# jantonguirao/nvImageCodec

Hardware: AMD Instinct MI355X
Metric: images/sec, batched 1920x1080 4:2:0 baseline JPEG decode to interleaved RGB u8 (higher is better)
Workload: dtype int32

## Files before the change

nvimagecodec_amd/csrc/gpu_huffman.hip:

```cpp
#include <hip/hip_runtime.h>

#include "gpu_huffman.h"
#include "huffman_gpu_core.h"

namespace hipjpeg {

namespace {

constexpr int kThreads = 256;

constexpr int kRowShift = kSubseqWords == 32 ? 5 : kSubseqWords == 16 ? 4 : kSubseqWords == 64 ? 6 : -1;
static_assert(kRowShift > 0, "subsequences of 512, 1024 or 2048 bits");

#define HJ_LDS __attribute__((address_space(3)))
#define HJ_GLOBAL __attribute__((address_space(1)))
typedef unsigned int u32x4 __attribute__((ext_vector_type(4)));

struct KSlot {
    int16_t* base;
    uint32_t stride_y, stride_x;
};

constexpr int kStagedExtra = 2;
constexpr int kRowWords = kSubseqWords + kStagedExtra;
// ... 58 lines not shown
        *(HJ_GLOBAL uint16_t*)(records + (off + 2 * min(i, (uint32_t)kRecSlots))) = (uint16_t)(pos - bit0);
    }
};
__device__ __forceinline__ SlotRecorder slot_recorder(uint16_t* records, const HuffImage& im, uint32_t j)
{
    SlotRecorder r;
    r.records = (HJ_GLOBAL char*)records;
    r.off = (im.first_subseq + j) * (uint32_t)(2 * kRecShorts);
    r.bit0 = j * kSubseqBits;
    return r;
}
__device__ __forceinline__ void put_mark(const SlotRecorder& r, uint32_t begin, uint32_t limit, uint32_t total_bits, uint32_t z0, const SubseqState& st)
{
    *(HJ_GLOBAL uint16_t*)(r.records + (r.off + 2 * kRecMark)) = (uint16_t)record_mark(begin, min(limit, total_bits), z0, st);
}

template <class Env>
__device__ __forceinline__ SubseqState walk_subsequence(bool rst, bool record, const HuffGeom& geom, const Env& env, uint32_t begin, uint32_t limit, int z,
                                                        int k, uint32_t boundary0, const SlotRecorder& rec)
{
    if (rst) return decode_subsequence<true>(geom, env, begin, limit, z, k, boundary0);
    return record ? decode_subsequence<false>(geom, env, begin, limit, z, k, 0, rec) : decode_subsequence<false>(geom, env, begin, limit, z, k);
}

template <int ROWS>
__device__ __forceinline__ void stage_rows(uint32_t* lds_stream, const HuffImage& im, int first_row)
{
    const int t = threadIdx.x;
    const HJ_GLOBAL uint32_t* g = (const HJ_GLOBAL uint32_t*)im.stream;
    const int nwords = (int)im.stream_words;
    const int w0 = (first_row + t) * kSubseqWords;
    constexpr int kGroups = kSubseqWords / 4;
    u32x4 v[kGroups];
    typedef unsigned int u32x2 __attribute__((ext_vector_type(2)));
    u32x2 tail;
    {
        const int gd = w0 + kSubseqWords;
        const int gc = min(max(gd, 0), (nwords - 1) & ~1);
        const u32x2 x = *(const HJ_GLOBAL u32x2*)(g + gc);
        tail = (gd >= 0 && gd < nwords) ? x : u32x2{~0u, ~0u};
    }
#pragma unroll
    for (int i = 0; i < kGroups; i++) {
        const int gd = w0 + i * 4;
        const int gc = min(max(gd, 0), (nwords - 1) & ~3);
        const u32x4 x = *(const HJ_GLOBAL u32x4*)(g + gc);
        v[i] = (gd >= 0 && gd < nwords) ? x : u32x4{~0u, ~0u, ~0u, ~0u};
    }
    HJ_LDS uint32_t* dst = (HJ_LDS uint32_t*)lds_stream + t;
#pragma unroll
    for (int i = 0; i < kGroups; i++) {
        dst[(4 * i + 0) * ROWS] = __builtin_bswap32(v[i].x);
        dst[(4 * i + 1) * ROWS] = __builtin_bswap32(v[i].y);
        dst[(4 * i + 2) * ROWS] = __builtin_bswap32(v[i].z);
        dst[(4 * i + 3) * ROWS] = __builtin_bswap32(v[i].w);
    }
    dst[(kSubseqWords + 0) * ROWS] = __builtin_bswap32(tail.x);
    dst[(kSubseqWords + 1) * ROWS] = __builtin_bswap32(tail.y);
}

template <int THREADS>
__device__ __forceinline__ void stage_pool(HJ_LDS uint16_t* pool, const HuffImage& im)
{
    const HJ_GLOBAL u32x4* gp = (const HJ_GLOBAL u32x4*)im.pool;
    const uint32_t npool = im.pool_words >> 3;
    for (uint32_t i = threadIdx.x; i < npool; i += THREADS) {
        const u32x4 x = gp[i];
        HJ_LDS uint32_t* lp = reinterpret_cast<HJ_LDS uint32_t*>(pool) + i * 4;
        lp[0] = x.x;
        lp[1] = x.y;
        lp[2] = x.z;
        lp[3] = x.w;
    }
}

__device__ __forceinline__ void stage_constants(uint32_t* tsel, KSlot* kslot, uint32_t* zzw, const HuffImage& im, bool with_addresses)
{
    const int t = threadIdx.x;
    if (t < 10) {
        const HuffK hk = im.k[t];
        tsel[t] = ((uint32_t)hk.tdc * 2) | ((uint32_t)hk.tac * 2 << 16);
        if (with_addresses) {
            KSlot s;
            s.base = im.coef[hk.comp & 3] + (size_t)hk.blk0 * 64;
            s.stride_y = hk.stride_y;
            s.stride_x = hk.stride_x;
            kslot[t] = s;
        }
    }
    if (zzw && t >= 64 && t < 80) {
        constexpr uint8_t zz[64] = HJ_ZIGZAG_DEVICE_TABLE;
        const int i = (t - 64) * 4;
        zzw[t - 64] = ((uint32_t)zz[i] | ((uint32_t)zz[i + 1] << 8) | ((uint32_t)zz[i + 2] << 16) | ((uint32_t)zz[i + 3] << 24)) << 1;
    }
}

__device__ __forceinline__ DevEnv make_env(WgShared& sh, HJ_LDS uint16_t* pool, uint32_t first, const HuffGeom& geom)
{
    DevEnv env;
    env.stream_base = (uint32_t)(uintptr_t)(HJ_LDS uint32_t*)sh.stream;
    env.word0 = (first - 1) * kSubseqWords;
    env.row_addr = env.stream_base;
    env.row_word0 = env.word0;
    env.pool = (uint32_t)(uintptr_t)pool;
    env.tsel = (const HJ_LDS uint32_t*)sh.tsel;
    env.boundaries = geom.boundaries;
    env.num_boundaries = geom.num_boundaries;
    return env;
}

__device__ __forceinline__ int compact_tasks(WgShared& sh, bool has, int value, int* task)
{
    const int t = threadIdx.x;
    const unsigned long long mask = __ballot(has);
    const int below = __popcll(mask & ((1ull << (t & 63)) - 1));
    if ((t & 63) == 0) sh.wave_count[t >> 6] = (uint32_t)__popcll(mask);
    __syncthreads();
    int base = 0, n = 0;
#pragma unroll
    for (int w = 0; w < kSyncThreads / 64; w++) {
        const int c = (int)sh.wave_count[w];
        if (w < (t >> 6)) base += c;
        n += c;
    }
    if (has) sh.queue[base + below] = (uint32_t)value;
    __syncthreads();
    *task = t < n ? (int)sh.queue[t] : -1;
    return n;
}

constexpr int kGatherGroups = 64;
__global__ __launch_bounds__(kThreads) void gather_raw_kernel(const HuffImage* __restrict__ images, const HuffUnit* __restrict__ units, int nunits)
{
    for (int ui = blockIdx.x; ui < nunits; ui += gridDim.x) {
        const HuffUnit u = units[ui];
        const HuffImage& im = images[u.image];
        const uint8_t* src = im.raw_src;
        if (!src) continue;
        const uint32_t begin = u.first * (uint32_t)kDestuffChunk;
        if (begin >= im.raw_bytes) continue;
        const uint32_t n = min((uint32_t)kDestuffChunk, im.raw_bytes - begin);
        const uint8_t* s = src + begin;
        uint8_t* d = const_cast<uint8_t*>(im.raw) + begin;
        typedef u32x4 __attribute__((aligned(1))) u32x4_unaligned;
        for (uint32_t i = threadIdx.x * 16u; i + 16u <= n; i += kThreads * 16u) *(HJ_GLOBAL u32x4*)(d + i) = *(const HJ_GLOBAL u32x4_unaligned*)(s + i);
        const uint32_t tail = n & ~15u;
        if (threadIdx.x < (n & 15u)) d[tail + threadIdx.x] = s[tail + threadIdx.x];
    }
}


__device__ __forceinline__ uint32_t zero_bytes(uint32_t v) { return ~(((v & 0x7F7F7F7Fu) + 0x7F7F7F7Fu) | v | 0x7F7F7F7Fu); }

__device__ __forceinline__ uint32_t stuffed_mask(uint32_t x, uint32_t prev, uint32_t next)
{
    const uint32_t ff_before = zero_bytes(~((x << 8) | prev));
    const uint32_t rst_x = zero_bytes((x & 0xF8F8F8F8u) ^ 0xD0D0D0D0u);
    const uint32_t second = (zero_bytes(x) | rst_x) & ff_before;
    const uint32_t after = (x >> 8) | (next << 24);
    const uint32_t first = zero_bytes(~x) & zero_bytes((after & 0xF8F8F8F8u) ^ 0xD0D0D0D0u);
    return second | first;
}

__device__ __forceinline__ uint32_t lane_masks(const uint8_t* p, bool has_prev, uint32_t m[16], uint32_t x[16])
{
    const uint4* q = reinterpret_cast<const uint4*>(p);
    uint32_t prev = has_prev ? p[-1] : 0u;
    uint32_t n = 0;
#pragma unroll
    for (int i = 0; i < 4; i++) {
        const uint4 v = q[i];
        x[4 * i + 0] = v.x;
        x[4 * i + 1] = v.y;
        x[4 * i + 2] = v.z;
        x[4 * i + 3] = v.w;
    }
    const uint32_t behind = p[64];
#pragma unroll
    for (int i = 0; i < 16; i++) {
        m[i] = stuffed_mask(x[i], prev, i < 15 ? (x[i < 15 ? i + 1 : 15] & 0xFFu) : behind);
        prev = x[i] >> 24;
        n += __popc(m[i]);
    }
    return n;
}

__device__ __forceinline__ uint32_t wg_sum(uint32_t v, uint32_t* scratch )
{
    for (int off = 32; off > 0; off >>= 1) v += __shfl_xor(v, off);
    if ((threadIdx.x & 63) == 0) scratch[threadIdx.x >> 6] = v;
    __syncthreads();
    const uint32_t total = scratch[0] + scratch[1] + scratch[2] + scratch[3];
    __syncthreads();
    return total;
}

__global__ __launch_bounds__(kThreads) void destuff_count_kernel(const HuffImage* __restrict__ images, const HuffUnit* __restrict__ units,
                                                                 uint32_t* __restrict__ drops)
{
    __shared__ uint32_t scratch[4];
    const HuffUnit u = units[blockIdx.x];
    const HuffImage& im = images[u.image];
    const uint32_t off = u.first * kDestuffChunk + threadIdx.x * 64;
    uint32_t n = 0;
    if (off < im.raw_bytes) {
        uint32_t m[16], x[16];
        const uint32_t pieces = min(4u, (im.raw_bytes - off + 15) / 16);
        if (pieces == 4) {
            n = lane_masks(im.raw + off, off > 0, m, x);
        } else {
            uint32_t prev = off > 0 ? im.raw[off - 1] : 0u;
            const uint32_t* words = reinterpret_cast<const uint32_t*>(im.raw + off);
            for (uint32_t i = 0; i < pieces * 4; i++) {
                const uint32_t w = words[i];
                n += __popc(stuffed_mask(w, prev, words[i + 1] & 0xFFu));
                prev = w >> 24;
            }
        }
    }
    const uint32_t total = wg_sum(n, scratch);
    if (threadIdx.x == 0) drops[im.first_chunk + u.first] = total;
}

__global__ __launch_bounds__(kThreads) void destuff_compact_kernel(HuffImage* __restrict__ images, const HuffUnit* __restrict__ units,
                                                                   const uint32_t* __restrict__ drops, unsigned int* __restrict__ counters)
{
    if (blockIdx.x == 0 && threadIdx.x < 64 && counters) counters[threadIdx.x] = 0u;
    __shared__ uint32_t scratch[4];
    __shared__ uint32_t wave_base[4];
    __shared__ uint32_t buf[kDestuffChunk / 4 + kDestuffChunk / 64 + 8];
    HJ_LDS uint8_t* bytes = (HJ_LDS uint8_t*)buf;
    const HuffUnit u = units[blockIdx.x];
    HuffImage& im = images[u.image];
    const int t = threadIdx.x;
    const uint32_t raw_bytes = im.raw_bytes;
    uint32_t before = 0;
    for (uint32_t c = t; c < u.first; c += kThreads) before += drops[im.first_chunk + c];
    before = wg_sum(before, scratch);
    const uint32_t chunk_begin = u.first * kDestuffChunk;
    const uint32_t chunk_len = min((uint32_t)kDestuffChunk, raw_bytes - chunk_begin);
    const uint32_t gout = chunk_begin - before;
    const uint32_t a = gout & 3;

    {
        const uint32_t pieces = (chunk_len + 15) / 16;
        const HJ_GLOBAL u32x4* src = (const HJ_GLOBAL u32x4*)(im.raw + chunk_begin);
        constexpr uint32_t kPiecesPerLane = kDestuffChunk / 16 / kThreads;
        u32x4 v[kPiecesPerLane];
#pragma unroll
        for (uint32_t i = 0; i < kPiecesPerLane; i++) v[i] = src[min(i * kThreads + t, pieces - 1)];
#pragma unroll
        for (uint32_t i = 0; i < kPiecesPerLane; i++) {
            const uint32_t q = i * kThreads + t, g = q * 4 + (q >> 2);
            const u32x4 x = q < pieces ? v[i] : u32x4{0x01010101u, 0x01010101u, 0x01010101u, 0x01010101u};
            buf[g] = x.x;
            buf[g + 1] = x.y;
            buf[g + 2] = x.z;
            buf[g + 3] = x.w;
        }
    }
    const uint32_t before_chunk = chunk_begin > 0 ? im.raw[chunk_begin - 1] : 0u;
    const uint32_t behind_chunk = chunk_len == (uint32_t)kDestuffChunk ? im.raw[chunk_begin + kDestuffChunk] : 0x01u;
    __syncthreads();

    const uint32_t off = chunk_begin + t * 64;
    uint32_t x[16];
    unsigned long long kept = 0;
    uint32_t n = 0, len = 0;
    if (off < raw_bytes) {
        len = min(64u, raw_bytes - off);
        const uint32_t pieces = (len + 15) / 16;
        uint32_t prev = t > 0 ? buf[(t - 1) * 17 + 15] >> 24 : before_chunk;
#pragma unroll
        for (uint32_t i = 0; i < 16; i++) x[i] = i < pieces * 4 ? buf[t * 17 + i] : 0x01010101u;
        const uint32_t behind = pieces == 4 ? (t < kThreads - 1 ? buf[(t + 1) * 17] & 0xFFu : behind_chunk) : 0x01u;
#pragma unroll
        for (uint32_t i = 0; i < 16; i++) {
            uint32_t w = x[i];
            uint32_t d = stuffed_mask(w, prev, i < 15 ? (x[i < 15 ? i + 1 : 15] & 0xFFu) : behind);
            prev = w >> 24;
            n += __popc(d);
            if (len < 64) {
                const uint32_t in = len > i * 4 ? min(len - i * 4, 4u) : 0u;
                if (in < 4) d |= 0x80808080u << (8 * in);
            }
            w = (d & 0x80000000u) ? (w & 0x00FFFFFFu) : w;
            w = (d & 0x00800000u) ? ((w & 0xFFFFu) | ((w >> 8) & 0xFF0000u)) : w;
            w = (d & 0x00008000u) ? ((w & 0xFFu) | ((w >> 8) & 0xFFFF00u)) : w;
            w = (d & 0x00000080u) ? (w >> 8) : w;
            x[i] = w;
            kept |= (unsigned long long)(4 - __popc(d)) << (3 * i);
        }
    }
    uint32_t incl = n;
    for (int d = 1; d < 64; d <<= 1) {
        const uint32_t v = __shfl_up(incl, d);
        if ((t & 63) >= d) incl += v;
    }
    if ((t & 63) == 63) wave_base[t >> 6] = incl;
    __syncthreads();
    uint32_t excl = incl - n;
    for (int w = 0; w < (t >> 6); w++) excl += wave_base[w];
    const uint32_t chunk_drops = wave_base[0] + wave_base[1] + wave_base[2] + wave_base[3];
    auto padded = [](uint32_t k) { return k + ((k >> 6) << 2); };
    const uint32_t o0 = a + t * 64 - excl, cnt0 = o0 & 3;
    uint32_t o = o0 & ~3u, cnt = cnt0;
    unsigned long long acc = 0;
    if (len) {
#pragma unroll
        for (uint32_t i = 0; i < 16; i++) {
            acc |= (unsigned long long)x[i] << (8 * cnt);
            cnt += (uint32_t)(kept >> (3 * i)) & 7u;
            if (cnt >= 4) {
                buf[(o >> 2) + (o >> 6)] = (uint32_t)acc;
                acc >>= 32;
                cnt -= 4;
                o += 4;
            }
        }
    }
    __syncthreads();
    {
        const uint32_t from = o == (o0 & ~3u) ? cnt0 : 0u;
#pragma unroll
        for (uint32_t b = 0; b < 3; b++)
            if (b >= from && b < cnt) bytes[padded(o + b)] = (uint8_t)((uint32_t)acc >> (8 * b));
    }
    __syncthreads();
    const uint32_t n_out = chunk_len - chunk_drops;
    uint8_t* dst = const_cast<uint8_t*>(im.stream) + (gout - a);
    const uint32_t first_full = a ? 1 : 0, end_full = (a + n_out) / 4;
    for (uint32_t d = first_full + t; d < end_full; d += kThreads) reinterpret_cast<uint32_t*>(dst)[d] = buf[d + (d >> 4)];
    if (t < 4) {
        if (a && (uint32_t)t >= a && (uint32_t)t < a + n_out) dst[t] = bytes[padded((uint32_t)t)];
        const uint32_t tail = max(end_full, first_full) * 4 + t;
        if (tail >= a && tail < a + n_out && tail >= 4 * first_full) dst[tail] = bytes[padded(tail)];
    }
    if (chunk_begin + chunk_len == raw_bytes) {
        const uint32_t total = raw_bytes - before - chunk_drops;
        const uint32_t padded = ((total + 3) & ~3u) + kStreamSlackBytes;
        uint8_t* s = const_cast<uint8_t*>(im.stream);
        if (total + t < padded) s[total + t] = 0xFF;
        if (t == 0) {
            im.total_bits = total * 8;
            im.num_subseq = (total * 8 + kSubseqBits - 1) / kSubseqBits;
            im.stream_words = padded / 4;
        }
    }
}

__global__ __launch_bounds__(kSyncThreads) void huff_sync_kernel(const HuffImage* __restrict__ images, const HuffUnit* __restrict__ units,
                                                             unsigned long long* __restrict__ states, unsigned long long* __restrict__ incoming,
                                                             unsigned int* __restrict__ counters, int first_pass, int max_rounds,
                                                             uint16_t* __restrict__ tail_tasks, uint32_t* __restrict__ tail_count, uint16_t* records)
{
    __shared__ WgShared sh;
    extern __shared__ uint16_t dyn_pool[];
    HJ_LDS uint16_t* pool = (HJ_LDS uint16_t*)dyn_pool;
    const HuffUnit u = units[blockIdx.x];
    const HuffImage& im = images[u.image];
    const HuffGeom geom = make_geom(im);
    const uint32_t nsub = (geom.total_bits + kSubseqBits - 1) / kSubseqBits;
    if (u.first >= nsub) return;
    unsigned long long* gstate = states + im.first_subseq;
    const int t = threadIdx.x;
    const uint32_t j = u.first - 1 + t;
    const bool owner = t >= 1 && j < nsub;
    const int n_rows = (int)min((uint32_t)kSyncThreads, nsub - u.first + 1);
    unsigned long long in_state = 0;
    if (!first_pass) {
        in_state = u.first ? __hip_atomic_load(&gstate[u.first - 1], __ATOMIC_RELAXED, __HIP_MEMORY_SCOPE_AGENT) & kSyncMask : 0ull;
        if (in_state == incoming[blockIdx.x]) return;
    }
    stage_rows<kSyncThreads>(sh.stream, im, (int)u.first - 1);
    stage_pool<kSyncThreads>(pool, im);
    stage_constants(sh.tsel, nullptr, nullptr, im, false);
    __syncthreads();

    DevEnv env = make_env(sh, pool, u.first, geom);
    const bool rst = im.restart_interval != 0;
    unsigned long long old_global = ~0ull;
    int task = -1;
    const bool recording = !rst;
    if (first_pass) {
        const unsigned long long assumed = (unsigned long long)j * kSubseqBits;
        unsigned long long mine = 0;
        if (owner || (t == 0 && u.first > 0)) {
            const uint32_t bidx0 = boundary0_of(im, j);
            env.set_row(t);
            mine = pack_state(walk_subsequence(rst, false, geom, env, j * kSubseqBits, (j + 1) * kSubseqBits, 0, 0, bidx0, SlotRecorder()));
        }
        sh.end[t] = mine;
        __syncthreads();
        if (owner && ((sh.end[t - 1] & kSyncMask) != assumed || recording)) task = t;
    } else {
        if (owner) old_global = gstate[j];
        sh.end[t] = t == 0 ? in_state : old_global;
        if (t == 1) task = 1;
    }
    int rounds = 0;
    for (int round = 0; round < kSyncThreads + 2; round++) {
        __syncthreads();
        rounds++;
        unsigned long long now = 0;
        bool moved = false;
        if (task >= 0) {
            const SubseqState p = unpack_state(sh.end[task - 1]);
            env.set_row(task);
            const uint32_t jt = u.first - 1 + task;
            const SlotRecorder rec = slot_recorder(records, im, jt);
            const SubseqState st = walk_subsequence(rst, recording, geom, env, p.end_bit, (jt + 1) * kSubseqBits, p.zk & 255, p.zk >> 8, boundary0_of(im, jt), rec);
            if (recording) put_mark(rec, p.end_bit, (jt + 1) * kSubseqBits, geom.total_bits, p.zk & 255, st);
            now = pack_state(st);
            moved = ((now ^ sh.end[task]) & kSyncMask) != 0;
        }
        __syncthreads();
        if (task >= 0) sh.end[task] = now;
        const int pending = compact_tasks(sh, moved && task + 1 < n_rows, task + 1, &task);
        if (pending == 0 || rounds >= max_rounds) {
            if (tail_count) {
                if (t < pending) tail_tasks[(size_t)blockIdx.x * kSyncThreads + t] = (uint16_t)task;
                if (t == 0) tail_count[blockIdx.x] = (uint32_t)pending;
            }
            break;
        }
    }
    __syncthreads();
    if (owner) {
        const unsigned long long mine = sh.end[t];
        if (mine != old_global) {
            __hip_atomic_store(&gstate[j], mine, __ATOMIC_RELAXED, __HIP_MEMORY_SCOPE_AGENT);
            if (t == n_rows - 1 && ((mine ^ old_global) & kSyncMask) != 0) atomicAdd(counters + (first_pass ? 1 : 0), 1u);
        }
    }
    if (t == 0) {
        incoming[blockIdx.x] = first_pass ? (sh.end[0] & kSyncMask) : in_state;
        atomicAdd(counters + (first_pass ? 2 : 4), (unsigned)rounds);
        atomicMax(counters + (first_pass ? 3 : 5), (unsigned)rounds);
    }
}

constexpr int kTailWaves = 4;
constexpr int kTailThreads = 64 * kTailWaves;
#ifndef HJ_TAIL_SLOTS
#define HJ_TAIL_SLOTS 32
#endif
constexpr int kTailSlots = HJ_TAIL_SLOTS;
static_assert(kTailSlots == 32 || kTailSlots == 64, "a power of two, at most one row buffer per lane");
constexpr int kTailRowWords = kSubseqWords + 4;

struct TailWave {
    uint32_t rows[kTailSlots * kTailRowWords];
    uint16_t list[2][kSyncThreads];
    uint32_t count[2];
};
struct TailShared {
    TailWave wave[kTailWaves];
    uint32_t tsel[10];
};

struct TailEnv {
    uint32_t row_base;
    uint32_t word0;
    uint32_t pool;
    const HJ_LDS uint32_t* tsel;
    const uint32_t* boundaries;
    uint32_t num_boundaries;
    __device__ __forceinline__ uint32_t boundary(uint32_t i) const { return load_boundary(boundaries, num_boundaries, i); }
    static constexpr uint32_t kCursorStep = (uint32_t)kTailSlots * 4u;
    __device__ __forceinline__ uint32_t cursor(uint32_t i) const { return row_base + (i - word0) * kCursorStep; }
    __device__ __forceinline__ uint32_t fetch(uint32_t c) const { return *(const HJ_LDS uint32_t*)(uintptr_t)c; }
    __device__ __forceinline__ uint32_t tables(int k) const { return tsel[k]; }
    __device__ __forceinline__ uint32_t lookup1(uint32_t t, uint32_t w) const
    {
        return *(const HJ_LDS uint16_t*)(uintptr_t)(pool + t + ((w >> (31 - kHuffFastBits)) & ((2u << kHuffFastBits) - 2)));
    }
// ... 444 lines not shown
    {
        const HJ_LDS KSlot* s = kslot + k;
        int16_t* base = s->base;
        const uint32_t sy = s->stride_y, sx = s->stride_x;
        return base + (size_t)(my * sy + mx * sx) * 64;
    }
    __device__ __forceinline__ int zigzag(int z) const { return zz[z]; }
    __device__ __forceinline__ void put(int byte_offset, int value) const { *(HJ_LDS int16_t*)(uintptr_t)(buf ^ (uint32_t)byte_offset) = (int16_t)value; }
};

__global__ __launch_bounds__(kBThreads, 4) void huff_blocks_kernel(HuffImage* __restrict__ images, const HuffUnit* __restrict__ units,
                                                                   uint32_t nunits, int32_t* __restrict__ group_sums)
{
    __shared__ BlockShared sh;
    extern __shared__ uint16_t dyn_pool[];
    HJ_LDS uint16_t* pool = (HJ_LDS uint16_t*)dyn_pool;
    const uint32_t per_team = gridDim.x / (uint32_t)kBTeams;
    const uint32_t unit0 = (blockIdx.x % per_team) * (uint32_t)kBTeams + blockIdx.x / per_team;
    if (unit0 >= nunits) return;
    const HuffUnit u0 = units[unit0];
    if ((u0.first / (uint32_t)kHuffMcusPerWg) % (uint32_t)kBTeams != 0) return;
    HuffImage& im = images[u0.image];
    const HuffGeom geom = make_geom(im);
    const uint32_t bpm = geom.blocks_per_mcu;
    const uint32_t nblocks = min(im.total_blocks, im.decoded_blocks);
    const uint32_t total_mcus = geom.mcus_x * geom.mcus_y;
    const int t = threadIdx.x, team = t / kBTeamThreads, tt = t % kBTeamThreads;
    const uint32_t first = u0.first + (uint32_t)team * kHuffMcusPerWg;
    const bool has_unit = first < total_mcus;
    const uint32_t b_first = first * bpm;
    const uint32_t mcus = has_unit && b_first < nblocks ? min((uint32_t)kHuffMcusPerWg, total_mcus - first) : 0u;
    const uint32_t items = mcus * bpm;
    if (t < 4 * kBTeams) sh.dc_sum[t >> 2][t & 3] = 0;
    if (t >= 32 && t < 42) sh.kcomp[t - 32] = im.k[t - 32].comp & 3;
    stage_pool<kBThreads>(pool, im);
    stage_constants(sh.tsel, sh.kslot, sh.zz, im, true);
    HJ_LDS u32x4* my_buf = (HJ_LDS u32x4*)&sh.blocks[t * kBlockBufBytes];
#pragma unroll
    for (int i = 0; i < kBlockBufBytes / 16; i++) my_buf[i] = u32x4{0u, 0u, 0u, 0u};
    __syncthreads();
    BlockEnv env;
    env.gstream = reinterpret_cast<const uint32_t*>(im.stream);
    env.gwords = im.stream_words;
    env.pool = (uint32_t)(uintptr_t)pool;
    env.buf = (uint32_t)(uintptr_t)(HJ_LDS uint8_t*)sh.blocks + (((uint32_t)t * kBlockBufBytes) | (((uint32_t)t & 7u) << 4));
    env.tsel = (const HJ_LDS uint32_t*)sh.tsel;
    env.kslot = (const HJ_LDS KSlot*)sh.kslot;
    env.zz = (const HJ_LDS uint8_t*)sh.zz;
    uint32_t err = 0;
    static_assert(kBTeamThreads % 64 == 0, "whole waves: lane t flushes the buffers of lanes (t & ~63) ...");
    for (uint32_t base = 0; base < items; base += kBTeamThreads) {
        wave_sync();
        const uint32_t item = base + tt;
        int16_t* dst = nullptr;
        if (item < items) {
            const uint32_t k = item / mcus, mcu = first + (item - k * mcus);
            const uint32_t b = mcu * bpm + k;
            if (b < nblocks) {
                const uint32_t my = mcu / geom.mcus_x, mx = mcu - my * geom.mcus_x;
                dst = env.block_ptr((int)k, mx, my);
                const uint32_t bpos = im.block_pos[b];
                if (geom.interval_blocks != 0 && k == 0 && b != 0 && b % geom.interval_blocks == 0 &&
                    bpos != load_boundary(geom.boundaries, geom.num_boundaries, b / geom.interval_blocks - 1))
                    err = 1;
                const int dc = decode_block(geom, env, bpos, (int)k, &err);
                ((HJ_GLOBAL int16_t*)geom.dc_diff)[b] = (int16_t)dc;
                atomicAdd(&sh.dc_sum[team][sh.kcomp[k]], (int)(int16_t)dc);
            }
        }
        wave_sync();
        const uint32_t dst_lo = (uint32_t)(uintptr_t)dst, dst_hi = (uint32_t)((uintptr_t)dst >> 32);
        const int lane = t & 63, chunk = t & 7;
        int16_t* p[8];
        u32x4 v[8];
#pragma unroll
        for (int i = 0; i < 8; i++) {
            const int src = 8 * i + (lane >> 3);
            const uint32_t lo = (uint32_t)__shfl((int)dst_lo, src, 64), hi = (uint32_t)__shfl((int)dst_hi, src, 64);
            p[i] = (int16_t*)(((uintptr_t)hi << 32) | lo);
        }
#pragma unroll
        for (int i = 0; i < 8; i++) {
            const int blk = (t & ~63) + 8 * i + (lane >> 3);
            v[i] = *(const HJ_LDS u32x4*)&sh.blocks[blk * kBlockBufBytes + ((chunk ^ (blk & 7)) << 4)];
        }
#pragma unroll
        for (int i = 0; i < 8; i++)
            if (p[i]) __builtin_nontemporal_store(v[i], (HJ_GLOBAL u32x4*)p[i] + chunk);
        if (base + kBTeamThreads < items) {
            wave_sync();
#pragma unroll
            for (int i = 0; i < 8; i++) my_buf[i] = u32x4{0u, 0u, 0u, 0u};
        }
    }
    if (err) im.status = 1;
    __syncthreads();
    if (has_unit && tt < 4) group_sums[(size_t)(unit0 + team) * 4 + tt] = sh.dc_sum[team][tt];
}

__global__ __launch_bounds__(kThreads) void huff_dcdiff_kernel(HuffImage* __restrict__ images, const HuffUnit* __restrict__ units,
                                                              int32_t* __restrict__ group_sums)
{
    __shared__ int32_t s_sum[4];
    __shared__ uint32_t s_tdc[10], s_comp[10];
    const HuffUnit u = units[blockIdx.x];
    HuffImage& im = images[u.image];
    const HuffGeom geom = make_geom(im);
    const uint32_t bpm = geom.blocks_per_mcu;
    const uint32_t nblocks = min(im.total_blocks, im.decoded_blocks);
    const uint32_t b_first = u.first * bpm;
    const int t = threadIdx.x;
    if (t < 4) s_sum[t] = 0;
    if (t >= 32 && t < 42) {
        s_tdc[t - 32] = im.k[t - 32].tdc;
        s_comp[t - 32] = im.k[t - 32].comp & 3;
    }
    __syncthreads();
    if (b_first < nblocks) {
        const uint32_t mcus = min((uint32_t)kHuffMcusPerWg, geom.mcus_x * geom.mcus_y - u.first);
        const uint32_t items = mcus * bpm;
        const HJ_GLOBAL uint32_t* g = (const HJ_GLOBAL uint32_t*)im.stream;
        const HJ_GLOBAL uint16_t* pool = (const HJ_GLOBAL uint16_t*)im.pool;
        const uint32_t gwords = im.stream_words;
        uint32_t err = 0;
        for (uint32_t item = t; item < items; item += kThreads) {
            const uint32_t b = b_first + item;
            if (b >= nblocks) break;
            const uint32_t k = item % bpm;
            const uint32_t bpos = im.block_pos[b];
            if (geom.interval_blocks != 0 && k == 0 && b != 0 && b % geom.interval_blocks == 0 &&
                bpos != load_boundary(geom.boundaries, geom.num_boundaries, b / geom.interval_blocks - 1))
                err = 1;
            const uint32_t i = bpos >> 5, sft = bpos & 31;
            const uint32_t w0 = i < gwords ? __builtin_bswap32(g[i]) : ~0u, w1 = i + 1 < gwords ? __builtin_bswap32(g[i + 1]) : ~0u;
            const uint32_t w = sft ? (w0 << sft) | (w1 >> (32 - sft)) : w0;
            uint32_t e = pool[s_tdc[k] + (w >> (32 - kHuffFastBits))];
            if ((e >> 9) == kZadvLong) e = pool[((e & 0x1FFu) << 6) + ((w >> (32 - kHuffFastBits - kHuffSubBits)) & ((1u << kHuffSubBits) - 1))];
            const uint32_t total = e & 31u, nb_raw = (e >> 5) & 15u;
            const bool bad = nb_raw >= total;
            const uint32_t nb = bad ? 0u : nb_raw;
            const uint32_t v = nb ? (w << (total - nb)) >> (32 - nb) : 0u;
            const uint32_t m = (1u << nb) - 1u;
            const int dc = (v << 1) <= m ? (int)v - (int)m : (int)v;
            if (bad || bpos + total > geom.total_bits) err = 1;
            ((HJ_GLOBAL int16_t*)geom.dc_diff)[b] = (int16_t)dc;
            atomicAdd(&s_sum[s_comp[k]], (int)(int16_t)dc);
        }
        if (err) im.status = 1;
    }
    __syncthreads();
    if (t < 4) group_sums[(size_t)blockIdx.x * 4 + t] = s_sum[t];
}

__global__ __launch_bounds__(kThreads) void huff_dc_group_kernel(const HuffImage* __restrict__ images, const HuffUnit* __restrict__ units,
                                                                 const int32_t* __restrict__ group_sums, const unsigned int* __restrict__ counters,
                                                                 unsigned int* __restrict__ verdicts)
{
    __shared__ int16_t s_diff[kHuffMcusPerWg * 10];
    __shared__ int s_base[4];
    const HuffUnit u = units[blockIdx.x];
    const HuffImage& im = images[u.image];
    if (verdicts) {
        if (blockIdx.x == 0 && threadIdx.x < kHuffVerdictCounters) verdicts[threadIdx.x] = counters[threadIdx.x];
        if (u.first == 0 && threadIdx.x == 64) verdicts[kHuffVerdictCounters + u.image] = huff_verdict(im.status, im.gave_up);
    }
    if (im.restart_interval != 0) return;
    const int t = threadIdx.x;
    const uint32_t bpm = im.blocks_per_mcu;
    const uint32_t total_mcus = im.mcus_x * im.mcus_y;
    const uint32_t mcus = min((uint32_t)kHuffMcusPerWg, total_mcus - u.first);
    const uint32_t n = mcus * bpm;
    const uint32_t g = u.first / kHuffMcusPerWg;
    if (t < 4) s_base[t] = 0;
    {
        const HJ_GLOBAL int16_t* diff = (const HJ_GLOBAL int16_t*)im.dc_diff + (size_t)u.first * bpm;
        for (uint32_t i = t; i < n; i += kThreads) s_diff[i] = diff[i];
    }
    __syncthreads();
    {
        const HJ_GLOBAL int32_t* sums = (const HJ_GLOBAL int32_t*)group_sums + (size_t)(blockIdx.x - g) * 4;
        int part = 0;
        for (uint32_t i = t; i < g * 4; i += kThreads) part += sums[i];
        if (part != 0) atomicAdd(&s_base[t & 3], part);
    }
    __syncthreads();
    const int c = t >> 6, lane = t & 63;
    if (c >= (int)im.ncomp) return;
    const uint32_t h = im.comp_h[c], v = im.comp_v[c], bpc = h * v, k0 = im.comp_k0[c];
    const uint32_t bw = im.blocks_w[c], mcus_x = im.mcus_x;
    HJ_GLOBAL int16_t* plane = (HJ_GLOBAL int16_t*)im.dc_plane[c];
    int run = s_base[c];
    const uint32_t nc = mcus * bpc;
    for (uint32_t s0 = 0; s0 < nc; s0 += 64) {
        const uint32_t s = s0 + lane;
        const bool live = s < nc;
        const uint32_t m = s / bpc, jj = s - m * bpc;
        int x = live ? (int)s_diff[m * bpm + k0 + jj] : 0;
#pragma unroll
        for (int d = 1; d < 64; d <<= 1) {
            const int y = __shfl_up(x, d, 64);
            if (lane >= d) x += y;
        }
        if (live) {
            const uint32_t mcu = u.first + m;
            const uint32_t my = mcu / mcus_x, mx = mcu - my * mcus_x;
            const uint32_t dy = jj / h, dx = jj - dy * h;
            plane[(my * v + dy) * bw + (mx * h + dx)] = (int16_t)(run + x);
        }
        run += __shfl(x, 63, 64);
    }
}

__global__ __launch_bounds__(kThreads) void huff_dc_kernel(const HuffImage* __restrict__ images, const HuffUnit* __restrict__ units)
{
    __shared__ int s_sum[kThreads];
    __shared__ int s_flag[kThreads];
    const HuffUnit u = units[blockIdx.x];
    const HuffImage& im = images[u.image];
    const int c = (int)u.first;
    const uint32_t h = im.comp_h[c], v = im.comp_v[c], bpc = h * v;
    const uint32_t bpm = im.blocks_per_mcu, k0 = im.comp_k0[c];
    const uint32_t mcus = im.mcus_x * im.mcus_y;
    const uint32_t n = mcus * bpc;
    HJ_GLOBAL int16_t* plane = (HJ_GLOBAL int16_t*)im.dc_plane[c];
    const HJ_GLOBAL int16_t* diff = (const HJ_GLOBAL int16_t*)im.dc_diff;
    const uint32_t bw = im.blocks_w[c], mcus_x = im.mcus_x;
    const uint32_t seg = im.restart_interval ? im.restart_interval * bpc : 0xFFFFFFFFu;
    const uint32_t per = (n + kThreads - 1) / kThreads;
    const uint32_t lo = min(n, threadIdx.x * per), hi = min(n, lo + per);
    auto index_of = [&](uint32_t s) {
        const uint32_t mcu = s / bpc;
        return mcu * bpm + k0 + (s - mcu * bpc);
    };
    constexpr int kBatch = 8;
    int sum = 0, flag = 0;
    uint32_t until = lo < hi ? (seg == 0xFFFFFFFFu ? 0xFFFFFFFFu : (seg - lo % seg) % seg) : 0xFFFFFFFFu;
    for (uint32_t s = lo; s < hi; s += kBatch) {
        int d[kBatch];
#pragma unroll
        for (int i = 0; i < kBatch; i++) d[i] = s + i < hi ? (int)diff[index_of(s + i)] : 0;
#pragma unroll
        for (int i = 0; i < kBatch; i++) {
            if (s + i < hi) {
                if (until == 0) {
                    sum = 0;
                    flag = 1;
                    until = seg;
                }
                until--;
            }
            sum += d[i];
        }
    }
    s_sum[threadIdx.x] = sum;
    s_flag[threadIdx.x] = flag;
    __syncthreads();
    for (int off = 1; off < kThreads; off <<= 1) {
        int a = 0, fa = 0;
        if (threadIdx.x >= (unsigned)off) {
            a = s_sum[threadIdx.x - off];
            fa = s_flag[threadIdx.x - off];
        }
        __syncthreads();
        if (threadIdx.x >= (unsigned)off && !s_flag[threadIdx.x]) {
            s_sum[threadIdx.x] += a;
            s_flag[threadIdx.x] = fa;
        }
        __syncthreads();
    }
    int run = threadIdx.x ? s_sum[threadIdx.x - 1] : 0;
    until = lo < hi ? (seg == 0xFFFFFFFFu ? 0xFFFFFFFFu : (seg - lo % seg) % seg) : 0xFFFFFFFFu;
    for (uint32_t s = lo; s < hi; s += kBatch) {
        int d[kBatch];
#pragma unroll
        for (int i = 0; i < kBatch; i++) d[i] = s + i < hi ? (int)diff[index_of(s + i)] : 0;
#pragma unroll
        for (int i = 0; i < kBatch; i++) {
            if (s + i < hi) {
                if (until == 0) {
                    run = 0;
                    until = seg;
                }
                until--;
                run += d[i];
                const uint32_t mcu = (s + i) / bpc, jj = (s + i) - mcu * bpc;
                const uint32_t my = mcu / mcus_x, mx = mcu - my * mcus_x;
                const uint32_t dy = jj / h, dx = jj - dy * h;
                plane[(my * v + dy) * bw + (mx * h + dx)] = (int16_t)run;
            }
        }
    }
}

}

int launch_gather_raw(const HuffImage* images, const HuffUnit* chunk_units, int nchunks, void* stream)
{
    if (nchunks <= 0) return 0;
    hipLaunchKernelGGL(gather_raw_kernel, dim3(min(nchunks, kGatherGroups)), dim3(kThreads), 0, (hipStream_t)stream, images, chunk_units, nchunks);
    return (int)hipGetLastError();
}

int launch_destuff(HuffImage* images, const HuffUnit* chunk_units, int nchunks, uint32_t* drops, bool count_on_device, unsigned int* counters,
                   void* stream)
{
    if (nchunks <= 0) return 0;
    if (count_on_device)
        hipLaunchKernelGGL(destuff_count_kernel, dim3(nchunks), dim3(kThreads), 0, (hipStream_t)stream, images, chunk_units, drops);
    hipLaunchKernelGGL(destuff_compact_kernel, dim3(nchunks), dim3(kThreads), 0, (hipStream_t)stream, images, chunk_units, drops, counters);
    return (int)hipGetLastError();
}

static bool ripple_in_tail_kernel()
{
    static const bool v = getenv("HIPJPEG_RIPPLE_IN_SYNC") == nullptr;
    return v;
}

int launch_huff_sync(HuffImage* images, const HuffUnit* units, int nunits, unsigned long long* states, unsigned long long* incoming,
                     unsigned int* changed, int first_pass, int max_rounds, uint16_t* tail_tasks, uint32_t* tail_count, uint16_t* records,
                     unsigned pool_bytes, void* stream, unsigned pass_id)
{
    if (nunits <= 0) return 0;
    const dim3 tail_grid((nunits + kTailWaves - 1) / kTailWaves);
    if (!first_pass && ripple_in_tail_kernel()) {
        hipLaunchKernelGGL(huff_tail_kernel<true>, tail_grid, dim3(kTailThreads), pool_bytes, (hipStream_t)stream, images, units, nunits, states, incoming,
                           changed, nullptr, nullptr, pass_id, records);
        return (int)hipGetLastError();
    }
    hipLaunchKernelGGL(huff_sync_kernel, dim3(nunits), dim3(kSyncThreads), pool_bytes, (hipStream_t)stream, images, units, states, incoming, changed,
                       first_pass, max_rounds, tail_tasks, tail_count, records);
    if (tail_count)
        hipLaunchKernelGGL(huff_tail_kernel<false>, tail_grid, dim3(kTailThreads), pool_bytes, (hipStream_t)stream, images, units, nunits, states, incoming,
                           changed, tail_tasks, tail_count, 0u, records);
    return (int)hipGetLastError();
}

int launch_huff_write(HuffImage* images, const HuffUnit* sync_units, int nsync_units, const HuffUnit* block_units, int nblock_units,
                      const unsigned long long* states, uint32_t* first_block, const uint16_t* records, uint32_t* walkers, int32_t* group_sums,
                      unsigned pool_bytes, void* stream, bool dc_only)
{
    if (nsync_units <= 0) return 0;
    hipLaunchKernelGGL(huff_copy_records_kernel, dim3(nsync_units), dim3(kSyncThreads), 0, (hipStream_t)stream, images, sync_units, states, first_block,
                       records, walkers);
    hipLaunchKernelGGL(huff_pos_kernel, dim3(nsync_units), dim3(kSyncThreads), pool_bytes, (hipStream_t)stream, images, sync_units, states, first_block,
                       records, walkers);
    if (nblock_units > 0) {
        if (dc_only)
            hipLaunchKernelGGL(huff_dcdiff_kernel, dim3(nblock_units), dim3(kThreads), 0, (hipStream_t)stream, images, block_units, group_sums);
        else
            hipLaunchKernelGGL(huff_blocks_kernel, dim3((nblock_units + kBTeams - 1) / kBTeams * kBTeams), dim3(kBThreads), pool_bytes, (hipStream_t)stream,
                               images, block_units, (uint32_t)nblock_units, group_sums);
    }
    return (int)hipGetLastError();
}

int launch_huff_dc(const HuffImage* images, const HuffUnit* rst_units, int nrst_units, const HuffUnit* block_units, int nblock_units,
                   const int32_t* group_sums, const unsigned int* counters, unsigned int* verdicts, void* stream)
{
    if (nblock_units > 0)
        hipLaunchKernelGGL(huff_dc_group_kernel, dim3(nblock_units), dim3(kThreads), 0, (hipStream_t)stream, images, block_units, group_sums, counters,
                           verdicts);
    if (nrst_units > 0) hipLaunchKernelGGL(huff_dc_kernel, dim3(nrst_units), dim3(kThreads), 0, (hipStream_t)stream, images, rst_units);
// ... 5 lines not shown
```

Before: 102,400.

## Skip restart-marker masks, use perm-based byte squeeze, restructure DC prefix scan

The destuff kernels now compute restart-marker masks only when the image has a restart interval; otherwise they check only FF00 stuffing. The per-word byte squeeze uses a precomputed v_perm selector table instead of chained conditional shifts, and 32-bit packing replaces the 64-bit accumulator. The DC group kernel now has each lane sum a run of MCUs sequentially before one wave scan, replacing repeated per-64-element wave scans with divisions. For 3-component images with a 128-multiple group size, the idle fourth wave helps with component 0. This adds complexity and more LDS synchronisation.

```diff
diff --git a/nvimagecodec_amd/csrc/gpu_huffman.hip b/nvimagecodec_amd/csrc/gpu_huffman.hip
--- a/nvimagecodec_amd/csrc/gpu_huffman.hip
+++ b/nvimagecodec_amd/csrc/gpu_huffman.hip
@@ -234,17 +234,24 @@
 
 __device__ __forceinline__ uint32_t zero_bytes(uint32_t v) { return ~(((v & 0x7F7F7F7Fu) + 0x7F7F7F7Fu) | v | 0x7F7F7F7Fu); }
 
-__device__ __forceinline__ uint32_t stuffed_mask(uint32_t x, uint32_t prev, uint32_t next)
-{
-    const uint32_t ff_before = zero_bytes(~((x << 8) | prev));
+__device__ __forceinline__ uint32_t stuffed_zero_mask(uint32_t x, uint32_t prev) { return zero_bytes(x | ~((x << 8) | prev)); }
+
+__device__ __forceinline__ uint32_t marker_mask(uint32_t x, uint32_t prev, uint32_t next)
+{
+    const uint32_t ff_x = zero_bytes(~x);
     const uint32_t rst_x = zero_bytes((x & 0xF8F8F8F8u) ^ 0xD0D0D0D0u);
-    const uint32_t second = (zero_bytes(x) | rst_x) & ff_before;
+    const uint32_t ff_before = (ff_x << 8) | (prev == 0xFFu ? 0x80u : 0u);
     const uint32_t after = (x >> 8) | (next << 24);
-    const uint32_t first = zero_bytes(~x) & zero_bytes((after & 0xF8F8F8F8u) ^ 0xD0D0D0D0u);
-    return second | first;
-}
-
-__device__ __forceinline__ uint32_t lane_masks(const uint8_t* p, bool has_prev, uint32_t m[16], uint32_t x[16])
+    return (rst_x & ff_before) | (ff_x & zero_bytes((after & 0xF8F8F8F8u) ^ 0xD0D0D0D0u));
+}
+
+__device__ __forceinline__ uint32_t stuffed_mask(uint32_t x, uint32_t prev, uint32_t next, bool markers)
+{
+    const uint32_t d = stuffed_zero_mask(x, prev);
+    return markers ? d | marker_mask(x, prev, next) : d;
+}
+
+__device__ __forceinline__ uint32_t lane_masks(const uint8_t* p, bool has_prev, bool markers, uint32_t m[16], uint32_t x[16])
 {
     const uint4* q = reinterpret_cast<const uint4*>(p);
     uint32_t prev = has_prev ? p[-1] : 0u;
@@ -260,7 +267,7 @@
     const uint32_t behind = p[64];
 #pragma unroll
     for (int i = 0; i < 16; i++) {
-        m[i] = stuffed_mask(x[i], prev, i < 15 ? (x[i < 15 ? i + 1 : 15] & 0xFFu) : behind);
+        m[i] = stuffed_mask(x[i], prev, i < 15 ? (x[i < 15 ? i + 1 : 15] & 0xFFu) : behind, markers);
         prev = x[i] >> 24;
         n += __popc(m[i]);
     }
@@ -284,18 +291,19 @@
     const HuffUnit u = units[blockIdx.x];
     const HuffImage& im = images[u.image];
     const uint32_t off = u.first * kDestuffChunk + threadIdx.x * 64;
+    const bool markers = im.restart_interval != 0;
     uint32_t n = 0;
     if (off < im.raw_bytes) {
         uint32_t m[16], x[16];
         const uint32_t pieces = min(4u, (im.raw_bytes - off + 15) / 16);
         if (pieces == 4) {
-            n = lane_masks(im.raw + off, off > 0, m, x);
+            n = lane_masks(im.raw + off, off > 0, markers, m, x);
         } else {
             uint32_t prev = off > 0 ? im.raw[off - 1] : 0u;
             const uint32_t* words = reinterpret_cast<const uint32_t*>(im.raw + off);
             for (uint32_t i = 0; i < pieces * 4; i++) {
                 const uint32_t w = words[i];
-                n += __popc(stuffed_mask(w, prev, words[i + 1] & 0xFFu));
+                n += __popc(stuffed_mask(w, prev, words[i + 1] & 0xFFu, markers));
                 prev = w >> 24;
             }
         }
@@ -311,11 +319,23 @@
     __shared__ uint32_t scratch[4];
     __shared__ uint32_t wave_base[4];
     __shared__ uint32_t buf[kDestuffChunk / 4 + kDestuffChunk / 64 + 8];
+    __shared__ uint32_t squeeze_sel[16];
     HJ_LDS uint8_t* bytes = (HJ_LDS uint8_t*)buf;
     const HuffUnit u = units[blockIdx.x];
     HuffImage& im = images[u.image];
     const int t = threadIdx.x;
+    if (t < 16) {
+        uint32_t sel = 0x0C0C0C0Cu, j = 0;
+#pragma unroll
+        for (uint32_t b = 0; b < 4; b++)
+            if (!((uint32_t)t >> b & 1u)) {
+                sel = (sel & ~(0xFFu << (8 * j))) | (b << (8 * j));
+                j++;
+            }
+        squeeze_sel[t] = sel;
+    }
     const uint32_t raw_bytes = im.raw_bytes;
+    const bool markers = im.restart_interval != 0;
     uint32_t before = 0;
     for (uint32_t c = t; c < u.first; c += kThreads) before += drops[im.first_chunk + c];
     before = wg_sum(before, scratch);
@@ -347,31 +367,37 @@
 
     const uint32_t off = chunk_begin + t * 64;
     uint32_t x[16];
-    unsigned long long kept = 0;
+    uint32_t gone[4] = {0, 0, 0, 0};
     uint32_t n = 0, len = 0;
     if (off < raw_bytes) {
         len = min(64u, raw_bytes - off);
         const uint32_t pieces = (len + 15) / 16;
-        uint32_t prev = t > 0 ? buf[(t - 1) * 17 + 15] >> 24 : before_chunk;
+        const uint32_t before_lane = t > 0 ? buf[(t - 1) * 17 + 15] >> 24 : before_chunk;
 #pragma unroll
         for (uint32_t i = 0; i < 16; i++) x[i] = i < pieces * 4 ? buf[t * 17 + i] : 0x01010101u;
-        const uint32_t behind = pieces == 4 ? (t < kThreads - 1 ? buf[(t + 1) * 17] & 0xFFu : behind_chunk) : 0x01u;
+        uint32_t d[16];
+        uint32_t prev = before_lane;
 #pragma unroll
         for (uint32_t i = 0; i < 16; i++) {
-            uint32_t w = x[i];
-            uint32_t d = stuffed_mask(w, prev, i < 15 ? (x[i < 15 ? i + 1 : 15] & 0xFFu) : behind);
-            prev = w >> 24;
-            n += __popc(d);
-            if (len < 64) {
-                const uint32_t in = len > i * 4 ? min(len - i * 4, 4u) : 0u;
-                if (in < 4) d |= 0x80808080u << (8 * in);
+            d[i] = stuffed_zero_mask(x[i], prev);
+            prev = x[i] >> 24;
+        }
+        if (markers) {
+            const uint32_t behind = pieces == 4 ? (t < kThreads - 1 ? buf[(t + 1) * 17] & 0xFFu : behind_chunk) : 0x01u;
+            prev = before_lane;
+#pragma unroll
+            for (uint32_t i = 0; i < 16; i++) {
+                d[i] |= marker_mask(x[i], prev, i < 15 ? (x[i < 15 ? i + 1 : 15] & 0xFFu) : behind);
+                prev = x[i] >> 24;
             }
-            w = (d & 0x80000000u) ? (w & 0x00FFFFFFu) : w;
-            w = (d & 0x00800000u) ? ((w & 0xFFFFu) | ((w >> 8) & 0xFF0000u)) : w;
-            w = (d & 0x00008000u) ? ((w & 0xFFu) | ((w >> 8) & 0xFFFF00u)) : w;
-            w = (d & 0x00000080u) ? (w >> 8) : w;
-            x[i] = w;
-            kept |= (unsigned long long)(4 - __popc(d)) << (3 * i);
+        }
+#pragma unroll
+        for (uint32_t i = 0; i < 16; i++) {
+            const uint32_t p = __popc(d[i]);
+            n += p;
+            gone[i / 5] |= p << (6 * (i % 5) + 3);
+            const uint32_t m = __builtin_amdgcn_udot4(d[i], 0x08040201u, 0u, false) >> 7;
+            x[i] = __builtin_amdgcn_perm(x[i], x[i], squeeze_sel[m]);
         }
     }
     uint32_t incl = n;
@@ -386,24 +412,24 @@
     const uint32_t chunk_drops = wave_base[0] + wave_base[1] + wave_base[2] + wave_base[3];
     auto padded = [](uint32_t k) { return k + ((k >> 6) << 2); };
     const uint32_t o0 = a + t * 64 - excl, cnt0 = o0 & 3;
-    uint32_t o = o0 & ~3u, cnt = cnt0;
-    unsigned long long acc = 0;
+    uint32_t slot = o0 >> 2, bits = 8 * cnt0, acc = 0;
     if (len) {
 #pragma unroll
         for (uint32_t i = 0; i < 16; i++) {
-            acc |= (unsigned long long)x[i] << (8 * cnt);
-            cnt += (uint32_t)(kept >> (3 * i)) & 7u;
-            if (cnt >= 4) {
-                buf[(o >> 2) + (o >> 6)] = (uint32_t)acc;
-                acc >>= 32;
-                cnt -= 4;
-                o += 4;
-            }
-        }
-    }
-    __syncthreads();
-    {
-        const uint32_t from = o == (o0 & ~3u) ? cnt0 : 0u;
+            const unsigned long long w = (unsigned long long)x[i] << bits;
+            const uint32_t p = (gone[i / 5] >> (6 * (i % 5))) & 63u;
+            const bool full = bits >= p;
+            acc |= (uint32_t)w;
+            if (full) buf[slot + (slot >> 4)] = acc;
+            acc = full ? (uint32_t)(w >> 32) : acc;
+            slot += full ? 1u : 0u;
+            bits = (bits - p) & 24u;
+        }
+    }
+    const uint32_t o = slot * 4, cnt = bits / 8;
+    __syncthreads();
+    {
+        const uint32_t from = slot == (o0 >> 2) ? cnt0 : 0u;
 #pragma unroll
         for (uint32_t b = 0; b < 3; b++)
             if (b >= from && b < cnt) bytes[padded(o + b)] = (uint8_t)((uint32_t)acc >> (8 * b));
@@ -1154,12 +1180,59 @@
     if (t < 4) group_sums[(size_t)blockIdx.x * 4 + t] = s_sum[t];
 }
 
+constexpr bool kDcSplit = kHuffMcusPerWg % 128 == 0;
+constexpr uint32_t kDcLaneMcus = kHuffMcusPerWg / 64;
+static_assert(kHuffMcusPerWg % 64 == 0, "huff_dc_group_kernel: the same number of MCUs for every lane of a wave");
+
+template <uint32_t BPC>
+__device__ __forceinline__ int dc_lane_total(const int16_t* d, uint32_t live, uint32_t bpc, uint32_t bpm)
+{
+    const uint32_t nb = BPC ? BPC : bpc;
+    int sum = 0;
+#pragma unroll
+    for (uint32_t q = 0; q < kDcLaneMcus; q++) {
+        if (q < live) {
+#pragma unroll
+            for (uint32_t jj = 0; jj < nb; jj++) sum += d[q * bpm + jj];
+        }
+    }
+    return sum;
+}
+
+template <uint32_t BPC>
+__device__ __forceinline__ void dc_lane_store(const int16_t* d, HJ_GLOBAL int16_t* plane, int run, uint32_t live, uint32_t bpc, uint32_t bpm,
+                                              uint32_t h, uint32_t v, uint32_t bw, uint32_t mx, uint32_t my, uint32_t mcus_x)
+{
+    const uint32_t nb = BPC ? BPC : bpc;
+#pragma unroll
+    for (uint32_t q = 0; q < kDcLaneMcus; q++) {
+        if (q < live) {
+            HJ_GLOBAL int16_t* p = plane + (my * v) * bw + mx * h;
+            uint32_t dx = 0;
+#pragma unroll
+            for (uint32_t jj = 0; jj < nb; jj++) {
+                run += d[q * bpm + jj];
+                p[dx] = (int16_t)run;
+                if (++dx == h) {
+                    dx = 0;
+                    p += bw;
+                }
+            }
+            if (++mx == mcus_x) {
+                mx = 0;
+                my++;
+            }
+        }
+    }
+}
+
 __global__ __launch_bounds__(kThreads) void huff_dc_group_kernel(const HuffImage* __restrict__ images, const HuffUnit* __restrict__ units,
                                                                  const int32_t* __restrict__ group_sums, const unsigned int* __restrict__ counters,
                                                                  unsigned int* __restrict__ verdicts)
 {
     __shared__ int16_t s_diff[kHuffMcusPerWg * 10];
     __shared__ int s_base[4];
+    __shared__ int s_half;
     const HuffUnit u = units[blockIdx.x];
     const HuffImage& im = images[u.image];
     if (verdicts) {
@@ -1169,48 +1242,60 @@
     if (im.restart_interval != 0) return;
     const int t = threadIdx.x;
     const uint32_t bpm = im.blocks_per_mcu;
-    const uint32_t total_mcus = im.mcus_x * im.mcus_y;
+    const uint32_t mcus_x = im.mcus_x, total_mcus = mcus_x * im.mcus_y;
     const uint32_t mcus = min((uint32_t)kHuffMcusPerWg, total_mcus - u.first);
     const uint32_t n = mcus * bpm;
     const uint32_t g = u.first / kHuffMcusPerWg;
     if (t < 4) s_base[t] = 0;
+    const HJ_GLOBAL int32_t* sums = (const HJ_GLOBAL int32_t*)group_sums + (size_t)(blockIdx.x - g) * 4;
+    int part = (uint32_t)t < g * 4 ? sums[t] : 0;
     {
         const HJ_GLOBAL int16_t* diff = (const HJ_GLOBAL int16_t*)im.dc_diff + (size_t)u.first * bpm;
-        for (uint32_t i = t; i < n; i += kThreads) s_diff[i] = diff[i];
-    }
-    __syncthreads();
-    {
-        const HJ_GLOBAL int32_t* sums = (const HJ_GLOBAL int32_t*)group_sums + (size_t)(blockIdx.x - g) * 4;
-        int part = 0;
-        for (uint32_t i = t; i < g * 4; i += kThreads) part += sums[i];
-        if (part != 0) atomicAdd(&s_base[t & 3], part);
-    }
-    __syncthreads();
-    const int c = t >> 6, lane = t & 63;
-    if (c >= (int)im.ncomp) return;
-    const uint32_t h = im.comp_h[c], v = im.comp_v[c], bpc = h * v, k0 = im.comp_k0[c];
-    const uint32_t bw = im.blocks_w[c], mcus_x = im.mcus_x;
-    HJ_GLOBAL int16_t* plane = (HJ_GLOBAL int16_t*)im.dc_plane[c];
-    int run = s_base[c];
-    const uint32_t nc = mcus * bpc;
-    for (uint32_t s0 = 0; s0 < nc; s0 += 64) {
-        const uint32_t s = s0 + lane;
-        const bool live = s < nc;
-        const uint32_t m = s / bpc, jj = s - m * bpc;
-        int x = live ? (int)s_diff[m * bpm + k0 + jj] : 0;
-#pragma unroll
-        for (int d = 1; d < 64; d <<= 1) {
-            const int y = __shfl_up(x, d, 64);
-            if (lane >= d) x += y;
-        }
-        if (live) {
-            const uint32_t mcu = u.first + m;
-            const uint32_t my = mcu / mcus_x, mx = mcu - my * mcus_x;
-            const uint32_t dy = jj / h, dx = jj - dy * h;
-            plane[(my * v + dy) * bw + (mx * h + dx)] = (int16_t)(run + x);
-        }
-        run += __shfl(x, 63, 64);
-    }
+        constexpr uint32_t kLoads = (kHuffMcusPerWg * 10 + kThreads - 1) / kThreads;
+        int16_t e[kLoads];
+#pragma unroll
+        for (uint32_t k = 0; k < kLoads; k++) e[k] = k * kThreads + t < n ? diff[k * kThreads + t] : (int16_t)0;
+#pragma unroll
+        for (uint32_t k = 0; k < kLoads; k++)
+            if (k * kThreads + t < n) s_diff[k * kThreads + t] = e[k];
+    }
+    for (uint32_t i = t + kThreads; i < g * 4; i += kThreads) part += sums[i];
+    __syncthreads();
+    if (part != 0) atomicAdd(&s_base[t & 3], part);
+    const int wave = t >> 6, lane = t & 63;
+    const bool split = kDcSplit && im.ncomp <= 3;
+    const bool helper = split && wave == 3;
+    const int c = helper ? 0 : wave;
+    const bool active = c < (int)im.ncomp;
+    const uint32_t per_lane = split && c == 0 ? kHuffMcusPerWg / 128 : kHuffMcusPerWg / 64;
+    const uint32_t m0 = ((helper ? 64u : 0u) + (uint32_t)lane) * per_lane;
+    const uint32_t live = active && m0 < mcus ? min(per_lane, mcus - m0) : 0u;
+    uint32_t h = 1, v = 1, bpc = 1, bw = 0, mx = 0, my = 0;
+    const int16_t* d = s_diff;
+    HJ_GLOBAL int16_t* plane = nullptr;
+    int x = 0;
+    if (active) {
+        h = im.comp_h[c], v = im.comp_v[c], bpc = h * v, bw = im.blocks_w[c];
+        d = s_diff + m0 * bpm + im.comp_k0[c];
+        plane = (HJ_GLOBAL int16_t*)im.dc_plane[c];
+        my = (u.first + m0) / mcus_x, mx = (u.first + m0) - my * mcus_x;
+        x = bpc == 1 ? dc_lane_total<1>(d, live, bpc, bpm) : bpc == 2 ? dc_lane_total<2>(d, live, bpc, bpm)
+          : bpc == 4 ? dc_lane_total<4>(d, live, bpc, bpm) : dc_lane_total<0>(d, live, bpc, bpm);
+    }
+    const int own = x;
+#pragma unroll
+    for (int s = 1; s < 64; s <<= 1) {
+        const int y = __shfl_up(x, s, 64);
+        if (lane >= s) x += y;
+    }
+    if (split && wave == 0 && lane == 63) s_half = x;
+    __syncthreads();
+    if (!active) return;
+    const int run = s_base[c] + (helper ? s_half : 0) + (x - own);
+    if (bpc == 1) dc_lane_store<1>(d, plane, run, live, bpc, bpm, h, v, bw, mx, my, mcus_x);
+    else if (bpc == 2) dc_lane_store<2>(d, plane, run, live, bpc, bpm, h, v, bw, mx, my, mcus_x);
+    else if (bpc == 4) dc_lane_store<4>(d, plane, run, live, bpc, bpm, h, v, bw, mx, my, mcus_x);
+    else dc_lane_store<0>(d, plane, run, live, bpc, bpm, h, v, bw, mx, my, mcus_x);
 }
 
 __global__ __launch_bounds__(kThreads) void huff_dc_kernel(const HuffImage* __restrict__ images, const HuffUnit* __restrict__ units)
```

After: 103,500, median of 6. 1.01x the previous value.
